# BCW-dot/PDE-based-Heston-Solver-GPU-accelerated

Hardware: AMD Instinct MI355X
Metric: grid-points x timesteps/sec (ADI sweep), 512x256 grid (higher is better)
Workload: dtype f64; 1 GPU; C2: European calls, Heston Douglas ADI, 512x256 grid, 1000 time steps, 256 strikes per GPU (85..115), HBM-resident inputs; m1=512, m2=256, instances_per_gpu=256, instances_total=256, parallelism=instances sharded over 1 GPU(s), no data-path collective

## Files before the change

pde_based_heston_solver_gpu_accelerated_amd/csrc/hadi_api.hip:

```cpp
#include "../../include/hadi.h"

#include <hip/hip_runtime.h>

#include <algorithm>
#include <climits>
#include <cmath>
#include <cstdarg>
#include <cstdio>
#include <cstdlib>
#include <cstring>
#include <string>
#include <vector>

#include "hadi_kernels.h"
#include "hadi_plan.h"

namespace {

struct DevBuf {
    void *p = nullptr;
    size_t cap = 0;
};

struct Ctx {
    int device = 0;
    hipStream_t stream = nullptr;
    hipEvent_t ev[4] = {nullptr, nullptr, nullptr, nullptr};
    std::vector<hipEvent_t> kev;
    int profiling = 0;
    int cu_count = 256;
    std::string name, arch;
    std::string err;
    hadi_timing timing{};
    DevBuf U, Y, LAM, U0, UT;
    DevBuf V, R1, C2;
    DevBuf rs_tab;
    DevBuf Uf, Yf;
    DevBuf scoef, b2row, rowc, a2i, pb, rinv, rwork, ipar, par8;
    DevBuf g_s, g_v, g_ds, g_dv;
    DevBuf src_v, src_dv, sel_a, sel_b, v0_i;
    DevBuf natU, natU0, natOut, prices, status;
    struct GraphEntry { std::string key; hipGraph_t graph; hipGraphExec_t exec; unsigned long long stamp; };
    std::vector<GraphEntry> graphs;
    unsigned long long graph_clock = 0;
    unsigned long long graph_captures = 0, graph_replays = 0, graph_drops = 0, graph_evictions = 0;
    int use_graph = 1;
    int graph_max_melems = 8;
    int use_small = 1;
    int small_seq = -1;
    int use_amp = 1;
    int device_vgrid = 1;
    int sub_batch = 1;
    int small_pairs = -1;
    int tile_il = 0;
    int col_prefetch = 0;
    int cs_strips = 1;
    int streams = 0;
    hipStream_t stream2 = nullptr;
    hipEvent_t fork_ev = nullptr, join_ev = nullptr;
    int last_nsub = 1;
    HadiTuning tune;
    hipEvent_t wait_ev = nullptr;
    DevBuf lm31;
    std::string last_path;
    DevBuf div_flag, div_amt, div_pct;
    DevBuf pay_mis;
    DevBuf order;
    int *err_host = nullptr, *err_dev = nullptr;
    char *pin = nullptr;
    size_t pin_cap = 0, pin_used = 0, pin_want = 0;
    int pin_dirty = 0;
    int debug_fault = 0;
    int team_launch = -1, team_failed = 0;
    DevBuf team;
};

struct DeviceGuard {
    int prev = -1;
    explicit DeviceGuard(int dev) {
        if (hipGetDevice(&prev) != hipSuccess) prev = -1;
        if (prev != dev) (void)hipSetDevice(dev);
        else prev = -1;
    }
    ~DeviceGuard() {
        if (prev >= 0) (void)hipSetDevice(prev);
    }
};

int fail(Ctx *c, int code, const char *fmt, ...) {
    char buf[512];
    va_list ap;
    va_start(ap, fmt);
    vsnprintf(buf, sizeof(buf), fmt, ap);
    va_end(ap);
    if (c) c->err = buf;
    return code;
}

#define HIP_TRY(c, call)                                                                          \
    do {                                                                                          \
        hipError_t e_ = (call);                                                                   \
        if (e_ != hipSuccess)                                                                     \
            return fail((c), HADI_ERR_HIP, "%s failed: %s (%s:%d)", #call, hipGetErrorString(e_), \
                        __FILE__, __LINE__);                                                      \
    } while (0)

void drop_graphs(Ctx *c) {
    for (auto &g : c->graphs) { (void)hipGraphExecDestroy(g.exec); (void)hipGraphDestroy(g.graph); }
    c->graph_drops += c->graphs.size();
    c->graphs.clear();
}

int ensure(Ctx *c, DevBuf &b, size_t bytes) {
    if (bytes <= b.cap) return HADI_OK;
    if (b.p) {
        HIP_TRY(c, hipStreamSynchronize(c->stream));
        drop_graphs(c);
        HIP_TRY(c, hipFree(b.p));
        b.p = nullptr;
        b.cap = 0;
    }
    const size_t want = bytes + bytes / 8 + 256;
    hipError_t e = hipMalloc(&b.p, want);
    if (e != hipSuccess) {
        b.p = nullptr;
        return fail(c, HADI_ERR_ALLOC, "hipMalloc(%zu bytes) failed: %s", want, hipGetErrorString(e));
    }
    b.cap = want;
    return HADI_OK;
}

template <class T>
T *ptr(DevBuf &b) {
    return static_cast<T *>(b.p);
}

void pin_rewind(Ctx *c) {
    if (c->pin_dirty && c->stream) (void)hipStreamSynchronize(c->stream);
    c->pin_dirty = 0;
    if (c->pin_want > c->pin_cap) {
        if (c->pin) (void)hipHostFree(c->pin);
        c->pin = nullptr; c->pin_cap = 0;
        const size_t want = c->pin_want + c->pin_want / 2 + 4096;
        void *q = nullptr;
        if (hipHostMalloc(&q, want, hipHostMallocDefault) == hipSuccess) { c->pin = static_cast<char *>(q); c->pin_cap = want; }
    }
    c->pin_used = 0;
    c->pin_want = 0;
}
void *pin_alloc(Ctx *c, size_t bytes) {
    const size_t need = (bytes + 63) & ~(size_t)63;
    c->pin_want += need;
    if (!c->pin || c->pin_used + need > c->pin_cap) return nullptr;
    void *q = c->pin + c->pin_used;
    c->pin_used += need;
    return q;
}
// ... 49 lines not shown
    int debug = 0, debug_step = 1;
};

template <int B, int G, int NG, int PD>
void launch_pass_a(const HadiPlan &pl, const HadiSweepArgs &a, int n, hipStream_t s, int mode = 0) {
    if (mode == 1)
        hipLaunchKernelGGL((hadi_pass_a<B, G, 4, NG, PD, false, 1>), dim3(pl.grid_a), dim3(64 * pl.W * G * NG), pl.smem_a, s, a, n);
    else if (mode == 2)
        hipLaunchKernelGGL((hadi_pass_a<B, G, 4, NG, PD, false, 2>), dim3(pl.grid_a), dim3(64 * pl.W * G * NG), pl.smem_a, s, a, n);
    else if (a.american)
        hipLaunchKernelGGL((hadi_pass_a<B, G, 4, NG, PD, true>), dim3(pl.grid_a), dim3(64 * pl.W * G * NG), pl.smem_a, s, a, n);
    else
        hipLaunchKernelGGL((hadi_pass_a<B, G, 4, NG, PD, false>), dim3(pl.grid_a), dim3(64 * pl.W * G * NG), pl.smem_a, s, a, n);
}

template <int B, int G, int NG, int PD>
void launch_pass_a_f32(const HadiPlan &pl, const HadiSweepArgs &a, int n, hipStream_t s) {
    const size_t ring_elems = (size_t)NG * ((PD + 1) * pl.W + 4) * pl.L.rowp;
    const size_t smem = pl.smem_a - ring_elems * (sizeof(double) - sizeof(float));
    hipLaunchKernelGGL((hadi_pass_a<B, G, 4, NG, PD, false, 0, float>), dim3(pl.grid_a), dim3(64 * pl.W * G * NG), smem, s, a, n);
}

template <int B, int G, int NG, int PD>
void launch_pass_a_amp(const HadiPlan &pl, const HadiSweepArgs &a, int n, hipStream_t s) {
    hipLaunchKernelGGL((hadi_pass_a<B, G, 4, NG, PD, 2>), dim3(pl.grid_a), dim3(64 * pl.W * G * NG),
                       pl.smem_a + (size_t)pl.L.rowp * sizeof(double), s, a, n);
}

template <class K>
hipError_t raise_lds_limit(K kernel) {
    return hipFuncSetAttribute(reinterpret_cast<const void *>(kernel), hipFuncAttributeMaxDynamicSharedMemorySize, 160 * 1024);
}
template <int B, int G, int NG, int PD>
hipError_t raise_pass_a() {
    hipError_t e = raise_lds_limit(hadi_pass_a<B, G, 4, NG, PD, false>);
    if (e == hipSuccess) e = raise_lds_limit(hadi_pass_a<B, G, 4, NG, PD, false, 1>);
    if (e == hipSuccess) e = raise_lds_limit(hadi_pass_a<B, G, 4, NG, PD, false, 2>);
    return e != hipSuccess ? e : raise_lds_limit(hadi_pass_a<B, G, 4, NG, PD, true>);
}
template <int B, int G, int NG, int PD, int SCH>
hipError_t raise_pass_a_sch() {
    hipError_t e = raise_lds_limit(hadi_pass_a_sch<B, G, 4, NG, PD, 1, SCH>);
    return e != hipSuccess ? e : raise_lds_limit(hadi_pass_a_sch<B, G, 4, NG, PD, 2, SCH>);
}
template <int SCH>
hipError_t raise_sch_lds_limits() {
    hipError_t e;
    if ((e = raise_pass_a_sch<1, 1, 1, 2, SCH>()) != hipSuccess) return e;
    if ((e = raise_pass_a_sch<2, 1, 1, 2, SCH>()) != hipSuccess) return e;
    if ((e = raise_pass_a_sch<4, 1, 1, 2, SCH>()) != hipSuccess) return e;
    if ((e = raise_pass_a_sch<8, 1, 1, 1, SCH>()) != hipSuccess) return e;
    if ((e = raise_pass_a_sch<8, 2, 1, 1, SCH>()) != hipSuccess) return e;
    if ((e = raise_lds_limit(hadi_pass_a_strip_sch<8, 1, 1, SCH>)) != hipSuccess) return e;
    if ((e = raise_lds_limit(hadi_pass_a_strip_sch<8, 1, 2, SCH>)) != hipSuccess) return e;
    if ((e = raise_lds_limit(hadi_pass_a_strip_sch<4, 1, 1, SCH>)) != hipSuccess) return e;
    if ((e = raise_lds_limit(hadi_pass_a_strip_sch<4, 1, 2, SCH>)) != hipSuccess) return e;
    if ((e = raise_lds_limit(hadi_pass_a_strip_sch<2, 1, 1, SCH>)) != hipSuccess) return e;
    if ((e = raise_lds_limit(hadi_pass_a_strip_sch<2, 1, 2, SCH>)) != hipSuccess) return e;
    return raise_lds_limit(hadi_pass_a_strip_sch<8, 2, 2, SCH>);
}
hipError_t raise_all_lds_limits() {
    hipError_t e;
    if ((e = raise_sch_lds_limits<HADI_SCH_MCS>()) != hipSuccess) return e;
    if ((e = raise_sch_lds_limits<HADI_SCH_HV>()) != hipSuccess) return e;
    if ((e = raise_pass_a<1, 1, 1, 2>()) != hipSuccess) return e;
    if ((e = raise_pass_a<2, 1, 1, 2>()) != hipSuccess) return e;
    if ((e = raise_pass_a<4, 1, 1, 2>()) != hipSuccess) return e;
    if ((e = raise_pass_a<8, 1, 1, 1>()) != hipSuccess) return e;
    if ((e = raise_pass_a<8, 2, 1, 1>()) != hipSuccess) return e;
    if ((e = raise_lds_limit(hadi_pass_a_strip<8, false>)) != hipSuccess) return e;
    if ((e = raise_lds_limit(hadi_pass_a_strip<8, true>)) != hipSuccess) return e;
    if ((e = raise_lds_limit(hadi_pass_a_strip<4, false>)) != hipSuccess) return e;
    if ((e = raise_lds_limit(hadi_pass_a_strip<4, true>)) != hipSuccess) return e;
    if ((e = raise_lds_limit(hadi_pass_a_strip<2, false>)) != hipSuccess) return e;
    if ((e = raise_lds_limit(hadi_pass_a_strip<2, true>)) != hipSuccess) return e;
    if ((e = raise_lds_limit(hadi_pass_a_strip<8, 2>)) != hipSuccess) return e;
    if ((e = raise_lds_limit(hadi_pass_a_strip<4, 2>)) != hipSuccess) return e;
    if ((e = raise_lds_limit(hadi_pass_a_strip<2, 2>)) != hipSuccess) return e;
    if ((e = raise_lds_limit(hadi_pass_a_pairs<0>)) != hipSuccess) return e;
    if ((e = raise_lds_limit(hadi_pass_a_pairs<1>)) != hipSuccess) return e;
    if ((e = raise_lds_limit(hadi_pass_a_pairs<2>)) != hipSuccess) return e;
    if ((e = raise_lds_limit(hadi_team_kernel<8>)) != hipSuccess) return e;
    if ((e = raise_lds_limit(hadi_team_kernel<4>)) != hipSuccess) return e;
    if ((e = raise_lds_limit(hadi_small_seq2_kernel<1>)) != hipSuccess) return e;
    if ((e = raise_lds_limit(hadi_small_seq2_kernel<2>)) != hipSuccess) return e;
    if ((e = raise_lds_limit(hadi_small_seq_kernel<1>)) != hipSuccess) return e;
    if ((e = raise_lds_limit(hadi_small_seq_kernel<2>)) != hipSuccess) return e;
    if ((e = raise_lds_limit(hadi_small_kernel<1, 4, false>)) != hipSuccess) return e;
    if ((e = raise_lds_limit(hadi_small_kernel<1, 4, true>)) != hipSuccess) return e;
    if ((e = raise_lds_limit(hadi_small_kernel<2, 4, false>)) != hipSuccess) return e;
    if ((e = raise_lds_limit(hadi_small_kernel<2, 4, true>)) != hipSuccess) return e;
    if ((e = raise_lds_limit(hadi_small_kernel<1, 8, false>)) != hipSuccess) return e;
    if ((e = raise_lds_limit(hadi_small_kernel<1, 8, true>)) != hipSuccess) return e;
    if ((e = raise_lds_limit(hadi_small_kernel<2, 8, false>)) != hipSuccess) return e;
    if ((e = raise_lds_limit(hadi_small_kernel<2, 8, true>)) != hipSuccess) return e;
    if ((e = raise_lds_limit(hadi_pass_b<8, false>)) != hipSuccess) return e;
    if ((e = raise_lds_limit(hadi_pass_b<8, true>)) != hipSuccess) return e;
    if ((e = raise_lds_limit(hadi_pass_b1<16, false>)) != hipSuccess) return e;
    if ((e = raise_lds_limit(hadi_pass_b2<16, double, HADI_B2_NPF(8)>)) != hipSuccess) return e;
    if ((e = raise_lds_limit(hadi_pass_b2<16, float, HADI_B2_NPF(4)>)) != hipSuccess) return e;
    if ((e = raise_lds_limit(hadi_pass_b<8, 2>)) != hipSuccess) return e;
    if ((e = raise_lds_limit(hadi_pass_b1<16, 2>)) != hipSuccess) return e;
    if ((e = raise_lds_limit(hadi_pass_a<1, 1, 4, 1, 2, 2>)) != hipSuccess) return e;
    if ((e = raise_lds_limit(hadi_pass_a<2, 1, 4, 1, 2, 2>)) != hipSuccess) return e;
    if ((e = raise_lds_limit(hadi_pass_a<4, 1, 4, 1, 2, 2>)) != hipSuccess) return e;
    if ((e = raise_lds_limit(hadi_pass_a<8, 1, 4, 1, 1, 2>)) != hipSuccess) return e;
    if ((e = raise_lds_limit(hadi_pass_a<8, 2, 4, 1, 1, 2>)) != hipSuccess) return e;
    if ((e = raise_lds_limit(hadi_pass_a_strip<8, false, float>)) != hipSuccess) return e;
    if ((e = raise_lds_limit(hadi_pass_a_strip<8, false, float, 2>)) != hipSuccess) return e;
    if ((e = raise_lds_limit(hadi_pass_a_strip<8, false, double, 2>)) != hipSuccess) return e;
    if ((e = raise_lds_limit(hadi_pass_a_strip<8, 1, double, 2>)) != hipSuccess) return e;
    if ((e = raise_lds_limit(hadi_pass_a_strip<8, 2, double, 2>)) != hipSuccess) return e;
    if ((e = raise_lds_limit(hadi_pass_b<8, false, float>)) != hipSuccess) return e;
    if ((e = raise_lds_limit(hadi_pass_b1<16, false, float>)) != hipSuccess) return e;
    if ((e = raise_lds_limit(hadi_pass_a<1, 1, 4, 1, 2, false, 0, float>)) != hipSuccess) return e;
    if ((e = raise_lds_limit(hadi_pass_a<2, 1, 4, 1, 2, false, 0, float>)) != hipSuccess) return e;
    if ((e = raise_lds_limit(hadi_pass_a<4, 1, 4, 1, 2, false, 0, float>)) != hipSuccess) return e;
    if ((e = raise_lds_limit(hadi_pass_a<8, 1, 4, 1, 1, false, 0, float>)) != hipSuccess) return e;
    if ((e = raise_lds_limit(hadi_pass_a<8, 2, 4, 1, 1, false, 0, float>)) != hipSuccess) return e;
    return raise_lds_limit(hadi_pass_b1<16, true>);
}

struct SubBatch { int off, cnt; HadiPlan pl; int lane; };
struct BatchPlan {
    std::vector<SubBatch> subs;
    bool two_streams = false;
    int fork_before = 0;
};
int plan_batches(Ctx *c, const SweepDesc &d, HadiPlan &pl, int state_bytes, bool seq_shape, BatchPlan &bp) {
    std::vector<SubBatch> &subs = bp.subs;
    bool &two_streams = bp.two_streams;
    int &fork_before = bp.fork_before;
    const bool no_strips = !(d.theta > 0.0) || d.r_d == d.r_f;
    auto plan_for = [&](int cnt, HadiPlan *q) {
        if (hadi_make_plan(d.m1, d.m2, cnt, 8 * c->cu_count, q, c->tune, state_bytes)) return 1;
        if (no_strips) q->use_strip = 0;
        return 0;
    };
    if (no_strips) pl.use_strip = 0;
    if (d.scheme == HADI_SCHEME_DOUGLAS && !d.debug && c->sub_batch && d.n > c->cu_count &&
        2ll * c->cu_count * pl.L.inst_stride * (long long)state_bytes >= (256ll << 20)) {
        const int cu = c->cu_count, full = d.n / cu, rem = d.n - full * cu;
        for (int k = 0; k < full; k++) subs.push_back(SubBatch{k * cu, cu, pl, 0});
        if (rem >= cu / 4) subs.push_back(SubBatch{full * cu, rem, pl, 0});
        else subs.back().cnt += rem;
        for (auto &sbt : subs)
            if (plan_for(sbt.cnt, &sbt.pl)) return fail(c, HADI_ERR_UNSUPPORTED, "plan failed");
        pl = subs[0].pl;
    } else {
        subs.push_back(SubBatch{0, d.n, pl, 0});
    }
    const bool streams_ok = d.scheme == HADI_SCHEME_DOUGLAS && !d.debug && !c->profiling && d.n >= 2 && !seq_shape;
    auto split_last = [&]() -> int {
        const SubBatch last = subs.back();
        const int h0 = (last.cnt + 1) / 2;
        subs.pop_back();
        subs.push_back(SubBatch{last.off, h0, last.pl, 0});
        subs.push_back(SubBatch{last.off + h0, last.cnt - h0, last.pl, 1});
        for (size_t k = subs.size() - 2; k < subs.size(); k++)
            if (plan_for(subs[k].cnt, &subs[k].pl)) return 1;
        return 0;
    };
    if (streams_ok && c->streams == 2) {
        if (subs.size() == 1) {
            if (split_last()) return fail(c, HADI_ERR_UNSUPPORTED, "plan failed");
        } else {
// ... 334 lines not shown
    sa.r_d = d.r_d; sa.r_f = d.r_f; sa.theta = d.theta;
    sa.scoef = ptr<double>(c->scoef); sa.b2row = ptr<double>(c->b2row); sa.rowc = ptr<double>(c->rowc);
    sa.a2i = ptr<double>(c->a2i); sa.pb = ptr<double>(c->pb); sa.rinv = ptr<double>(c->rinv);
    sa.rwork = ptr<double>(c->rwork); sa.ipar = ptr<HadiInstPar>(c->ipar);
    hipLaunchKernelGGL(hadi_setup_kernel, dim3(d.n), dim3(256), 0, s, sa);

    const size_t tot = (size_t)L.inst_stride * d.n;
    hipLaunchKernelGGL(hadi_pack_kernel, dim3(grid1d(tot)), dim3(256), 0, s, L, d.n, d.n_src, d.d_natU, ptr<double>(c->U));
    if (american) {
        hipLaunchKernelGGL(hadi_pack_kernel, dim3(grid1d(tot)), dim3(256), 0, s, L, d.n, d.n_src,
                           d.d_natU0 ? d.d_natU0 : d.d_natU, ptr<double>(c->U0));
        HIP_TRY(c, hipMemsetAsync(c->LAM.p, 0, st, s));
        if ((rc = ensure(c, c->pay_mis, sizeof(int) * n))) return rc;
        HIP_TRY(c, hipMemsetAsync(c->pay_mis.p, 0, sizeof(int) * n, s));
        hipLaunchKernelGGL(hadi_payoff_shape_kernel, dim3(grid1d(tot)), dim3(256), 0, s, L, d.n, ptr<double>(c->U0), ptr<int>(c->pay_mis));
    }
    bool amp = false;
    const bool takes_small_path = c->use_small && !c->profiling && !cs && !f32 && !d.debug && (american ? pl.smem_small_am : pl.smem_small_eu) > 0;
    if (american && c->use_amp && !cs && !takes_small_path && !d.debug && !seq_shape) {
        std::vector<int> mis(d.n);
        HIP_TRY(c, hipMemcpyAsync(mis.data(), c->pay_mis.p, sizeof(int) * n, hipMemcpyDeviceToHost, s));
        HIP_TRY(c, hipStreamSynchronize(s));
        amp = true;
        for (int k = 0; k < d.n; k++) amp = amp && mis[k] == 0;
    }
    HIP_TRY(c, hipGetLastError());

    if (f32) {
        hipLaunchKernelGGL(hadi_narrow_kernel, dim3(grid1d(tot)), dim3(256), 0, s, L, ptr<double>(c->U), ptr<float>(c->Uf), tot);
        HIP_TRY(c, hipMemsetAsync(c->Yf.p, 0, st / 2, s));
    }
    HadiSweepArgs a;
    a.U = ptr<double>(c->U); a.Y = ptr<double>(c->Y);
    if (f32) {
        a.U = reinterpret_cast<double *>(c->Uf.p);
        a.Y = reinterpret_cast<double *>(c->Yf.p);
    }
    a.LAM = american ? ptr<double>(c->LAM) : nullptr;
    a.U0 = american ? ptr<double>(c->U0) : nullptr;
    a.pay_mis = american ? ptr<int>(c->pay_mis) : nullptr;
    a.scoef = ptr<double>(c->scoef); a.b2row = ptr<double>(c->b2row); a.rowc = ptr<double>(c->rowc);
    a.pb = ptr<double>(c->pb); a.rinv = ptr<double>(c->rinv); a.ipar = ptr<HadiInstPar>(c->ipar);
    a.L = L; a.n_inst = d.n; a.R = pl.R; a.ntiles = pl.ntiles; a.ctiles = pl.ctiles; a.btpw = pl.btpw; a.bgroups = pl.bgroups;
    a.american = american ? 1 : 0; a.pos_m1 = pl.pos_m1;
    a.tile_il = c->tile_il;
    a.RS = pl.RS; a.sblocks = pl.sblocks;
    a.err = c->err_dev; a.debug = c->debug_fault;
    a.R1 = (cs || pl.row_seq) ? ptr<double>(c->R1) : nullptr;
    a.C2 = cs ? ptr<double>(c->C2) : nullptr;
    a.rs_tab = pair_tab ? ptr<double>(c->rs_tab) : nullptr;
    HadiSweepArgs av = a;
    if (cs) av.U = ptr<double>(c->V);

    const bool prof = c->profiling != 0 && !d.debug;
    if (prof) {
        const size_t need = (size_t)4 * d.Nmax * nsub;
        while (c->kev.size() < need) {
            hipEvent_t e;
            HIP_TRY(c, hipEventCreate(&e));
            c->kev.push_back(e);
        }
    }
    auto shift = [&](HadiSweepArgs x, int o, int cnt, const HadiPlan &sp) {
        x.n_inst = cnt; x.R = sp.R; x.ntiles = sp.ntiles; x.ctiles = sp.ctiles; x.btpw = sp.btpw; x.bgroups = sp.bgroups;
        x.RS = sp.RS; x.sblocks = sp.sblocks;
        const size_t so = (size_t)o * L.inst_stride;
        if (f32) {
            x.U = reinterpret_cast<double *>(reinterpret_cast<float *>(x.U) + so);
            x.Y = reinterpret_cast<double *>(reinterpret_cast<float *>(x.Y) + so);
        } else {
            x.U += so;
            x.Y += so;
        }
        if (x.LAM) x.LAM += so;
        if (x.U0) x.U0 += so;
        if (x.pay_mis) x.pay_mis += o;
        if (x.R1) x.R1 += so;
        if (x.C2) x.C2 += so;
        if (x.rs_tab) x.rs_tab += (size_t)o * L.nrows * 128;
        x.scoef += (size_t)o * pl.n_scoef; x.b2row += (size_t)o * pl.n_b2row; x.rowc += (size_t)o * pl.n_rowc;
        x.pb += (size_t)o * pl.n_pb; x.rinv += (size_t)o * pl.n_rinv; x.ipar += o;
        return x;
    };
    const HadiSweepArgs a_all = a, av_all = av;
    bool forked = false;
    auto enqueue_body = [&](hipStream_t q0) -> int {
      const int n_first = d.debug ? d.debug_step : 1, n_last = d.debug ? d.debug_step : d.Nmax;
      for (int sb = 0; sb < nsub; sb++) {
        if (two_streams && sb == fork_before) {
            HIP_TRY(c, hipEventRecord(c->fork_ev, q0));
            HIP_TRY(c, hipStreamWaitEvent(c->stream2, c->fork_ev, 0));
            forked = true;
        }
        hipStream_t q = (two_streams && subs[sb].lane) ? c->stream2 : q0;
        const int o = subs[sb].off, nsb = subs[sb].cnt;
        const HadiPlan &pl = subs[sb].pl;
        const size_t so = (size_t)o * L.inst_stride;
        const HadiSweepArgs a = shift(a_all, o, nsb, pl), av = shift(av_all, o, nsb, pl);
        const size_t tot = (size_t)L.inst_stride * nsb, st = tot * sizeof(double);
        double *const Ub = ptr<double>(c->U) + so, *const LAMb = american ? ptr<double>(c->LAM) + so : nullptr;
        double *const U0b = american ? ptr<double>(c->U0) + so : nullptr, *const UTb = dividend ? ptr<double>(c->UT) + so : nullptr;
        const int ev0 = 4 * sb * d.Nmax;
        if (pair_tab && pl.use_strip) {
            HadiSweepArgs at = a;
            at.U = Ub;
            const size_t sm = (size_t)4 * HADI_STRIP_NS(8, 2, 8) * L.rowp * sizeof(double) + ((size_t)4 * 64 * 8 * 2 + (size_t)4 * 16) * sizeof(double);
            hipLaunchKernelGGL((hadi_pass_a_strip<8, 0, double, 2, 3>), dim3(pl.grid_as), dim3(512), sm, q, at, 1);
        }
        for (int nstep = n_first; nstep <= n_last; nstep++) {
            const bool xstep = amp && (nstep == 1 || (have_div && div_step[nstep]));
            if (xstep && nstep > 1)
                hipLaunchKernelGGL(hadi_am_materialise_kernel, dim3(grid1d(tot)), dim3(256), 0, q, L, nsb, a.ipar, U0b, Ub, LAMb, pl.pos_m1);
            if (have_div && div_step[nstep]) {
                if (f32)
                    hipLaunchKernelGGL(hadi_widen_kernel, dim3(grid1d(tot)), dim3(256), 0, q, L, reinterpret_cast<const float *>(a.U), Ub, tot);
                HIP_TRY(c, hipMemcpyAsync(UTb, Ub, st, hipMemcpyDeviceToDevice, q));
                const size_t npts = (size_t)nsb * L.nrows * (L.m1 + 1);
                hipLaunchKernelGGL(hadi_dividend_kernel, dim3(grid1d(npts)), dim3(256), 0, q, L, nsb, a.ipar,
                                   d.d_vec_s + (size_t)o * (L.m1 + 1), UTb, Ub, ptr<int>(c->div_flag) + (size_t)o * flag_stride,
                                   flag_stride, nstep, ptr<double>(c->div_amt), ptr<double>(c->div_pct));
                if (f32)
                    hipLaunchKernelGGL(hadi_narrow_kernel, dim3(grid1d(tot)), dim3(256), 0, q, L, Ub, reinterpret_cast<float *>(a.U), tot);
            }
            if (prof) HIP_TRY(c, hipEventRecord(c->kev[ev0 + 4 * (nstep - 1) + 0], q));
            const PassEnv env{pl, L, nsb, q, nstep, american, amp, xstep, f32, c->col_prefetch, c->cs_strips, d.scheme};
            auto row_pass = [&](const HadiSweepArgs &ar, int mode) { launch_row_pass(env, ar, mode); };
            auto col_pass = [&](const HadiSweepArgs &ar) { launch_col_pass(env, ar); };
            if (d.debug == 2) {
                HIP_TRY(c, hipMemcpyAsync(a.Y, a.U, f32 ? st / 2 : st, hipMemcpyDeviceToDevice, q));
                col_pass(a);
                break;
            }
            row_pass(a, cs ? 1 : 0);
            if (d.debug == 1) break;
            if (prof) {
                HIP_TRY(c, hipEventRecord(c->kev[ev0 + 4 * (nstep - 1) + 1], q));
                HIP_TRY(c, hipEventRecord(c->kev[ev0 + 4 * (nstep - 1) + 2], q));
            }
            col_pass(cs ? av : a);
            if (prof) HIP_TRY(c, hipEventRecord(c->kev[ev0 + 4 * (nstep - 1) + 3], q));
            if (cs) {
                row_pass(av, 2);
                col_pass(a);
            }
            if (xstep)
                hipLaunchKernelGGL(hadi_am_dematerialise_kernel, dim3(grid1d(tot)), dim3(256), 0, q, L, nsb, a.ipar, U0b, Ub, LAMb);
        }
        if (amp)
            hipLaunchKernelGGL(hadi_am_materialise_kernel, dim3(grid1d(tot)), dim3(256), 0, q, L, nsb, a.ipar, U0b, Ub, LAMb, pl.pos_m1);
      }
      return HADI_OK;
    };
    auto enqueue_loop = [&](hipStream_t q0) -> int {
      forked = false;
      const int rcb = enqueue_body(q0);
      if (forked) {
          const hipError_t e1 = hipEventRecord(c->join_ev, c->stream2);
          const hipError_t e2 = e1 == hipSuccess ? hipStreamWaitEvent(q0, c->join_ev, 0) : e1;
          if (!rcb && e2 != hipSuccess) return fail(c, HADI_ERR_HIP, "joining the second stream failed: %s", hipGetErrorString(e2));
      }
      return rcb;
    };

    const size_t smem_small = american ? pl.smem_small_am : pl.smem_small_eu;
    const bool seq = takes_small_path && !american && (c->small_seq > 0 || (c->small_seq < 0 && d.n > c->cu_count));
    const size_t smem_seq = (size_t)hadi_small_seq_layout(L.m1, L.nrows).total * sizeof(double);
    const bool seq2 = seq && L.nrows <= 32 && 2 * smem_seq <= (size_t)160 * 1024 &&
                      (c->small_pairs > 0 || (c->small_pairs < 0 && d.n > 2 * c->cu_count && 2 * d.n <= 9 * c->cu_count));
    if (takes_small_path) {
        {
            char buf[192];
            if (seq2)
                std::snprintf(buf, sizeof buf, "hadi_small_seq2_kernel<%d>: whole time loop in one launch, two instances per wavefront, lines solved sequentially in LDS (2 x %zu B)", L.B, smem_seq);
            else if (seq)
                std::snprintf(buf, sizeof buf, "hadi_small_seq_kernel<%d>: whole time loop in one launch, one wavefront per instance, lines solved sequentially in LDS (%zu B)", L.B, smem_seq);
            else
                std::snprintf(buf, sizeof buf, "hadi_small_kernel<%d,%d,%s>: whole time loop in one launch, instance resident in LDS (%zu B)", L.B,
                              (c->tune.small_waves ? c->tune.small_waves : (d.n <= 2 * c->cu_count ? 8 : 4)) == 8 ? 8 : 4, american ? "AM" : "EU", smem_small);
            c->last_path = buf;
        }
        HadiSmallArgs sm;
        sm.div_flag = nullptr; sm.div_amounts = nullptr; sm.div_pcts = nullptr; sm.vec_s = d.d_vec_s; sm.Nmax = d.Nmax;
        sm.order = nullptr;
        if (!d.uniform_steps) {
            std::vector<int> order(d.n);
            for (int k = 0; k < d.n; k++) order[k] = k;
            std::stable_sort(order.begin(), order.end(), [&](int x, int y) {
                return d.par8[(size_t)x * 8 + 5] > d.par8[(size_t)y * 8 + 5];
            });
            if ((rc = ensure(c, c->order, sizeof(int) * n))) return rc;
            if ((rc = stage_to_device(c, c->order.p, order.data(), sizeof(int) * n))) return rc;
            sm.order = ptr<int>(c->order);
        }
        sm.flag_stride = flag_stride;
        if (have_div) {
            sm.div_flag = ptr<int>(c->div_flag); sm.div_amounts = ptr<double>(c->div_amt); sm.div_pcts = ptr<double>(c->div_pct);
        }
        HIP_TRY(c, hipEventRecord(c->ev[1], s));
        const int sw = c->tune.small_waves ? c->tune.small_waves : (d.n <= 2 * c->cu_count ? 8 : 4);
        if (seq2) {
            if (L.B == 1) hipLaunchKernelGGL((hadi_small_seq2_kernel<1>), dim3((d.n + 1) / 2), dim3(64), 2 * smem_seq, s, a, sm);
            else hipLaunchKernelGGL((hadi_small_seq2_kernel<2>), dim3((d.n + 1) / 2), dim3(64), 2 * smem_seq, s, a, sm);
        } else if (seq) {
            if (L.B == 1) hipLaunchKernelGGL((hadi_small_seq_kernel<1>), dim3(d.n), dim3(64), smem_seq, s, a, sm);
            else hipLaunchKernelGGL((hadi_small_seq_kernel<2>), dim3(d.n), dim3(64), smem_seq, s, a, sm);
        } else if (sw == 8) {
            if (L.B == 1) {
                if (american) hipLaunchKernelGGL((hadi_small_kernel<1, 8, true>), dim3(d.n), dim3(512), smem_small, s, a, sm);
                else hipLaunchKernelGGL((hadi_small_kernel<1, 8, false>), dim3(d.n), dim3(512), smem_small, s, a, sm);
            } else {
                if (american) hipLaunchKernelGGL((hadi_small_kernel<2, 8, true>), dim3(d.n), dim3(512), smem_small, s, a, sm);
                else hipLaunchKernelGGL((hadi_small_kernel<2, 8, false>), dim3(d.n), dim3(512), smem_small, s, a, sm);
            }
        } else if (L.B == 1) {
            if (american) hipLaunchKernelGGL((hadi_small_kernel<1, 4, true>), dim3(d.n), dim3(256), smem_small, s, a, sm);
            else hipLaunchKernelGGL((hadi_small_kernel<1, 4, false>), dim3(d.n), dim3(256), smem_small, s, a, sm);
        } else {
            if (american) hipLaunchKernelGGL((hadi_small_kernel<2, 4, true>), dim3(d.n), dim3(256), smem_small, s, a, sm);
            else hipLaunchKernelGGL((hadi_small_kernel<2, 4, false>), dim3(d.n), dim3(256), smem_small, s, a, sm);
        }
        HIP_TRY(c, hipGetLastError());
        HIP_TRY(c, hipEventRecord(c->ev[2], s));
        return HADI_OK;
    }

    c->last_path = describe_streaming_path(c, pl, bp, american, amp, d.scheme, f32);
    c->last_nsub = nsub;
    HIP_TRY(c, hipEventRecord(c->ev[1], s));
    const bool team_shape = d.n <= 8 && L.G == 1 && (L.B == 8 || L.B == 4) && L.P <= 8 && !seq_shape && (d.variant == HADI_EU || d.variant == HADI_DIV) && !cs && !f32 &&
                            !d.debug && !prof && d.theta > 0.0 && d.r_d != d.r_f && c->cu_count == 256;
    const bool pinned = c->tune.strip >= 0 || c->tune.row_tile > 0 || c->tune.col_groups > 0 || c->tune.strip_blocks > 0;
    if (team_shape && (c->team_launch > 0 || (c->team_launch < 0 && !c->team_failed && !pinned))) {
        if ((rc = ensure(c, c->team, 512 * sizeof(int)))) return rc;
        HIP_TRY(c, hipMemsetAsync(c->team.p, 0, 512 * sizeof(int), s));
        HadiTeamArgs ta;
        ta.form = ptr<int>(c->team); ta.bar = ptr<int>(c->team) + 64; ta.nb = c->cu_count / 8; ta.N = d.Nmax;
        ta.div_flag = have_div ? ptr<int>(c->div_flag) : nullptr; ta.flag_stride = flag_stride;
        ta.div_amounts = have_div ? ptr<double>(c->div_amt) : nullptr; ta.div_pcts = have_div ? ptr<double>(c->div_pct) : nullptr;
        ta.vec_s = d.d_vec_s;
        ta.stamps = reinterpret_cast<unsigned long long *>(ptr<int>(c->team) + 384);
        const size_t smem = ((size_t)4 * 64 * L.B + hadi_pb_mf_doubles(L.P) + (size_t)L.P * HADI_LC * HADI_PBW +
                             (have_div ? (size_t)(L.m1 + 2) + (size_t)8 * L.rowp : 0)) * sizeof(double) + 64;
        if (L.B == 8) hipLaunchKernelGGL((hadi_team_kernel<8>), dim3(c->cu_count), dim3(512), smem, s, a, ta);
        else hipLaunchKernelGGL((hadi_team_kernel<4>), dim3(c->cu_count), dim3(512), smem, s, a, ta);
        HIP_TRY(c, hipGetLastError());
        HIP_TRY(c, hipStreamSynchronize(s));
        const int deverr = __atomic_exchange_n(c->err_host, 0, __ATOMIC_ACQ_REL);
        if (!deverr) {
            char buf[200];
            std::snprintf(buf, sizeof buf, "hadi_team_kernel<%d>: whole time loop in one launch, every instance resident in one XCD's L2 (teams of %d blocks)",
                          L.B, ta.nb);
            c->last_path = buf;
            HIP_TRY(c, hipEventRecord(c->ev[2], s));
            return HADI_OK;
        }
        if (deverr & ~HADI_DEVERR_TEAM) __atomic_fetch_or(c->err_host, deverr & ~HADI_DEVERR_TEAM, __ATOMIC_RELAXED);
        c->team_failed = 1;
        hipLaunchKernelGGL(hadi_pack_kernel, dim3(grid1d(tot)), dim3(256), 0, s, L, d.n, d.n_src, d.d_natU, ptr<double>(c->U));
        HIP_TRY(c, hipMemsetAsync(c->Y.p, 0, st, s));
        c->last_path += " (after a failed instance-resident launch)";
    }
    const bool graphable = c->use_graph && !prof && !d.debug && (long long)d.n * L.inst_stride <= ((long long)c->graph_max_melems << 20);
    if (graphable) {
        std::string key;
        auto put = [&](const void *p_, size_t nbytes) { key.append(static_cast<const char *>(p_), nbytes); };
        {
            const void *pa[HADI_SWEEP_ARGS_NPTRS], *pv[HADI_SWEEP_ARGS_NPTRS];
            hadi_sweep_args_ptrs(a, pa);
            hadi_sweep_args_ptrs(av, pv);
            const void *own[] = {c->U.p, c->LAM.p, c->U0.p, c->UT.p, c->div_flag.p, c->div_amt.p, c->div_pct.p, d.d_vec_s};
            const int ints[] = {a.debug, a.L.m1, a.L.m2, a.L.B, a.L.G, a.L.P, a.n_inst, a.R, a.ntiles, a.ctiles, a.btpw, a.bgroups,
                                a.american, a.pos_m1, d.scheme, d.prec, (int)amp, (int)two_streams, nsub, pl.row_seq, pl.col_seq, pl.use_pairs, pl.use_strip, pl.RS, pl.sblocks, pl.grid_as, pl.grid_a, pl.grid_b, pl.block_b, pl.W, (int)pl.smem_a, (int)pl.smem_b};
            put(pa, sizeof(pa));
            put(pv, sizeof(pv));
            put(own, sizeof(own));
            put(ints, sizeof(ints));
        }
        for (const auto &sbt : subs) {
            const HadiPlan &q = sbt.pl;
            const int geo[] = {c->col_prefetch, c->cs_strips, c->tile_il, sbt.lane, fork_before, sbt.off, sbt.cnt, q.R, q.ntiles, q.grid_a, (int)q.smem_a, q.use_strip, q.use_pairs, q.RS, q.sblocks, q.grid_as,
                               (int)q.smem_as, q.ctiles, q.btpw, q.bgroups, q.grid_b, q.block_b, (int)q.smem_b, q.row_seq, q.col_seq, q.W, q.NG, q.PD};
            put(geo, sizeof(geo));
        }
        put(&d.Nmax, sizeof(int)); put(&d.dt0, sizeof(double));
        put(&d.variant, sizeof(int));
        if (have_div) {
            put(&flag_stride, sizeof(int));
            put(div_step.data(), div_step.size());
        }
        Ctx::GraphEntry *hit = nullptr;
        for (auto &g : c->graphs)
            if (g.key == key) { hit = &g; break; }
        if (!hit) {
            if (c->graphs.size() >= 8) {
                size_t lru = 0;
                for (size_t k = 1; k < c->graphs.size(); k++)
                    if (c->graphs[k].stamp < c->graphs[lru].stamp) lru = k;
                (void)hipGraphExecDestroy(c->graphs[lru].exec);
                (void)hipGraphDestroy(c->graphs[lru].graph);
                c->graphs.erase(c->graphs.begin() + lru);
                c->graph_evictions++;
            }
            hipGraph_t graph = nullptr;
            hipGraphExec_t exec = nullptr;
            HIP_TRY(c, hipStreamBeginCapture(s, hipStreamCaptureModeThreadLocal));
            const int rcl = enqueue_loop(s);
            hipError_t ec = hipStreamEndCapture(s, &graph);
            if (rcl || ec != hipSuccess) {
                if (graph) (void)hipGraphDestroy(graph);
                if (rcl) return rcl;
            }
            HIP_TRY(c, ec);
            HIP_TRY(c, hipGraphInstantiate(&exec, graph, nullptr, nullptr, 0));
            c->graphs.push_back(Ctx::GraphEntry{key, graph, exec, 0});
            hit = &c->graphs.back();
            c->graph_captures++;
        } else {
            c->graph_replays++;
        }
        hit->stamp = ++c->graph_clock;
        HIP_TRY(c, hipGraphLaunch(hit->exec, s));
    } else {
        const int rcl = enqueue_loop(s);
        if (rcl) return rcl;
    }
    HIP_TRY(c, hipGetLastError());
    HIP_TRY(c, hipEventRecord(c->ev[2], s));
    if (f32)
        hipLaunchKernelGGL(hadi_widen_kernel, dim3(grid1d(tot)), dim3(256), 0, s, L, ptr<float>(c->Uf), ptr<double>(c->U), tot);
    return HADI_OK;
}

int finish_timing(Ctx *c, const SweepDesc &d, const HadiPlan &pl) {
    hipStream_t s = c->stream;
    HIP_TRY(c, hipEventRecord(c->ev[3], s));
    HIP_TRY(c, hipStreamSynchronize(s));
    c->pin_dirty = 0;
    const int deverr = __atomic_exchange_n(c->err_host, 0, __ATOMIC_ACQ_REL);
    float ms = 0;
    hadi_timing &t = c->timing;
    t = hadi_timing{};
    HIP_TRY(c, hipEventElapsedTime(&ms, c->ev[0], c->ev[1])); t.setup_ms = ms;
    HIP_TRY(c, hipEventElapsedTime(&ms, c->ev[1], c->ev[2])); t.sweep_ms = ms;
    HIP_TRY(c, hipEventElapsedTime(&ms, c->ev[2], c->ev[3])); t.finish_ms = ms;
    long long ps = 0;
    const long long m = (long long)(d.m1 + 1) * (d.m2 + 1);
    for (int k = 0; k < d.n; k++) ps += m * (long long)d.par8[(size_t)k * 8 + 5];
    t.point_steps = ps;
    if (c->profiling && !d.debug && (int)c->kev.size() >= 4 * d.Nmax * c->last_nsub) {
        for (int k = 0; k < d.Nmax * c->last_nsub; k++) {
            HIP_TRY(c, hipEventElapsedTime(&ms, c->kev[4 * k], c->kev[4 * k + 1])); t.pass_a_ms += ms;
            HIP_TRY(c, hipEventElapsedTime(&ms, c->kev[4 * k + 2], c->kev[4 * k + 3])); t.pass_b_ms += ms;
        }
        t.pass_a_launches = (long long)d.Nmax * c->last_nsub;
        t.pass_b_launches = (long long)d.Nmax * c->last_nsub;
    }
    (void)pl;
    if (deverr)
        return fail(c, HADI_ERR_INTERNAL, "device-side failure 0x%x during the sweep%s: the results of this call are invalid", deverr,
                    (deverr & HADI_DEVERR_RENDEZVOUS) ? " (a pair rendezvous of a two-wavefront row ran out of polls)" : "");
    return HADI_OK;
}

int to_device(Ctx *c, int memspace, const double *src, size_t count, DevBuf &buf, const double **out) {
// ... 351 lines not shown
        case HADI_ERR_NOT_ON_GRID: return "S_0 is not a grid node";
        case HADI_ERR_NO_DEVICE: return "no usable gfx950 GPU (libhadi has no CPU path)";
        case HADI_ERR_ALLOC: return "device allocation failed";
        case HADI_ERR_INTERNAL: return "device-side failure reported by a kernel (results invalid)";
        default: return "unknown";
    }
}

int hadi_create(hadi_ctx **out, int device_id) {
    if (!out) return HADI_ERR_INVALID;
    *out = nullptr;
    int count = 0;
    if (hipGetDeviceCount(&count) != hipSuccess || count < 1) return HADI_ERR_NO_DEVICE;
    if (device_id < 0 || device_id >= count) return HADI_ERR_INVALID;
    DeviceGuard guard(device_id);
    hipDeviceProp_t prop;
    if (hipGetDeviceProperties(&prop, device_id) != hipSuccess) return HADI_ERR_HIP;
    if (std::strncmp(prop.gcnArchName, "gfx950", 6) != 0) return HADI_ERR_NO_DEVICE;
    Ctx *c = new Ctx;
    c->device = device_id;
    c->cu_count = prop.multiProcessorCount > 0 ? prop.multiProcessorCount : 256;
    c->name = prop.name;
    c->arch = prop.gcnArchName;
    bool ok = hipStreamCreateWithFlags(&c->stream, hipStreamNonBlocking) == hipSuccess;
    ok = ok && hipStreamCreateWithFlags(&c->stream2, hipStreamNonBlocking) == hipSuccess;
    ok = ok && hipEventCreateWithFlags(&c->fork_ev, hipEventDisableTiming) == hipSuccess;
    ok = ok && hipEventCreateWithFlags(&c->join_ev, hipEventDisableTiming) == hipSuccess;
    ok = ok && raise_all_lds_limits() == hipSuccess;
    for (auto &e : c->ev) ok = ok && hipEventCreate(&e) == hipSuccess;
    ok = ok && hipEventCreateWithFlags(&c->wait_ev, hipEventDisableTiming) == hipSuccess;
    ok = ok && hipHostMalloc(reinterpret_cast<void **>(&c->err_host), 64, hipHostMallocMapped | hipHostMallocCoherent) == hipSuccess;
    if (ok) {
        c->pin_want = (size_t)1 << 20;
        pin_rewind(c);
        *c->err_host = 0;
        ok = hipHostGetDevicePointer(reinterpret_cast<void **>(&c->err_dev), c->err_host, 0) == hipSuccess;
    }
    if (!ok) {
        release_handle(c);
        return HADI_ERR_HIP;
    }
    *out = reinterpret_cast<hadi_ctx *>(c);
    return HADI_OK;
}

int hadi_destroy(hadi_ctx *ctx) {
    Ctx *c = reinterpret_cast<Ctx *>(ctx);
    if (!c) return HADI_OK;
    DeviceGuard guard(c->device);
    release_handle(c);
    return HADI_OK;
}

const char *hadi_last_error(const hadi_ctx *ctx) {
    const Ctx *c = reinterpret_cast<const Ctx *>(ctx);
    return c ? c->err.c_str() : "null handle";
}

int hadi_set_profiling(hadi_ctx *ctx, int enabled) {
    Ctx *c = reinterpret_cast<Ctx *>(ctx);
    if (!c) return HADI_ERR_INVALID;
    c->profiling = enabled ? 1 : 0;
    return HADI_OK;
}

int hadi_set_tuning(hadi_ctx *ctx, const char *key, int value) {
    Ctx *c = reinterpret_cast<Ctx *>(ctx);
    if (!c || !key) return HADI_ERR_INVALID;
    if (!std::strcmp(key, "graph")) c->use_graph = value ? 1 : 0;
    else if (!std::strcmp(key, "small_grid")) c->use_small = value ? 1 : 0;
    else if (!std::strcmp(key, "small_seq")) c->small_seq = value < 0 ? -1 : (value ? 1 : 0);
    else if (!std::strcmp(key, "american_p")) c->use_amp = value ? 1 : 0;
    else if (!std::strcmp(key, "device_vgrid")) c->device_vgrid = value ? 1 : 0;
    else if (!std::strcmp(key, "sub_batch")) c->sub_batch = value ? 1 : 0;
    else if (!std::strcmp(key, "small_pairs")) c->small_pairs = value < 0 ? -1 : (value ? 1 : 0);
    else if (!std::strcmp(key, "streams")) c->streams = value == 2 ? 2 : (value == 1 ? 1 : 0);
    else if (!std::strcmp(key, "col_prefetch")) c->col_prefetch = value ? 1 : 0;
    else if (!std::strcmp(key, "cs_strips")) c->cs_strips = (value >= 0 && value <= 3) ? value : 1;
    else if (!std::strcmp(key, "graph_max_melems")) c->graph_max_melems = value > 0 ? value : 0;
    else if (!std::strcmp(key, "tile_interleave")) c->tile_il = value ? 1 : 0;
    else if (!std::strcmp(key, "strip")) c->tune.strip = value < 0 ? -1 : (value ? 1 : 0);
    else if (!std::strcmp(key, "debug_fault")) c->debug_fault = value;
    else if (!std::strcmp(key, "team_launch")) { c->team_launch = value < 0 ? -1 : (value ? 1 : 0); c->team_failed = 0; }
    else if (!std::strcmp(key, "row_tile")) c->tune.row_tile = value > 0 ? value : 0;
    else if (!std::strcmp(key, "strip_blocks")) c->tune.strip_blocks = value > 0 ? value : 0;
    else if (!std::strcmp(key, "pair_strips")) c->tune.pair_strips = value < 0 ? -1 : (value ? 1 : 0);
    else if (!std::strcmp(key, "col_groups")) c->tune.col_groups = value > 0 ? value : 0;
    else if (!std::strncmp(key, "model_", 6)) {
        struct { const char *k; int HadiTuning::*f; } const tab[] = {
            {"model_strip_row_ns", &HadiTuning::strip_row_ns}, {"model_ring_row_ps", &HadiTuning::ring_row_ps}, {"model_ring_fixed_ns", &HadiTuning::ring_fixed_ns},
            {"model_pstrip_row_ns", &HadiTuning::pstrip_row_ns}, {"model_pring_row_ps", &HadiTuning::pring_row_ps}, {"model_pring_fixed_ns", &HadiTuning::pring_fixed_ns}};
        bool hit = false;
        for (auto &e : tab)
            if (!std::strcmp(key, e.k)) { if (value < 1) return fail(c, HADI_ERR_INVALID, "%s must be positive", key); c->tune.*(e.f) = value; hit = true; }
        if (!hit) return fail(c, HADI_ERR_INVALID, "unknown tuning key '%s'", key);
    }
    else if (!std::strcmp(key, "small_waves")) {
        if (value != 0 && value != 4 && value != 8) return fail(c, HADI_ERR_INVALID, "small_waves must be 0, 4 or 8");
        c->tune.small_waves = value;
    } else if (!std::strcmp(key, "graph_captures") || !std::strcmp(key, "graph_replays") || !std::strcmp(key, "graph_drops") ||
               !std::strcmp(key, "graph_evictions")) {
        return fail(c, HADI_ERR_INVALID, "'%s' is a read-only counter", key);
    } else return fail(c, HADI_ERR_INVALID, "unknown tuning key '%s'", key);
    return HADI_OK;
}

int hadi_get_tuning(const hadi_ctx *ctx, const char *key, int *value) {
    const Ctx *c = reinterpret_cast<const Ctx *>(ctx);
    if (!c || !key || !value) return HADI_ERR_INVALID;
    if (!std::strcmp(key, "graph")) *value = c->use_graph;
    else if (!std::strcmp(key, "small_grid")) *value = c->use_small;
    else if (!std::strcmp(key, "small_seq")) *value = c->small_seq;
    else if (!std::strcmp(key, "american_p")) *value = c->use_amp;
    else if (!std::strcmp(key, "device_vgrid")) *value = c->device_vgrid;
    else if (!std::strcmp(key, "sub_batch")) *value = c->sub_batch;
    else if (!std::strcmp(key, "small_pairs")) *value = c->small_pairs;
    else if (!std::strcmp(key, "streams")) *value = c->streams;
    else if (!std::strcmp(key, "col_prefetch")) *value = c->col_prefetch;
    else if (!std::strcmp(key, "cs_strips")) *value = c->cs_strips;
    else if (!std::strcmp(key, "graph_max_melems")) *value = c->graph_max_melems;
    else if (!std::strcmp(key, "tile_interleave")) *value = c->tile_il;
    else if (!std::strcmp(key, "strip")) *value = c->tune.strip;
    else if (!std::strcmp(key, "debug_fault")) *value = c->debug_fault;
    else if (!std::strcmp(key, "team_launch")) *value = c->team_failed ? -2 : c->team_launch;
    else if (!std::strcmp(key, "row_tile")) *value = c->tune.row_tile;
    else if (!std::strcmp(key, "strip_blocks")) *value = c->tune.strip_blocks;
    else if (!std::strcmp(key, "pair_strips")) *value = c->tune.pair_strips;
    else if (!std::strcmp(key, "col_groups")) *value = c->tune.col_groups;
    else if (!std::strcmp(key, "model_strip_row_ns")) *value = c->tune.strip_row_ns;
    else if (!std::strcmp(key, "model_ring_row_ps")) *value = c->tune.ring_row_ps;
    else if (!std::strcmp(key, "model_ring_fixed_ns")) *value = c->tune.ring_fixed_ns;
    else if (!std::strcmp(key, "model_pstrip_row_ns")) *value = c->tune.pstrip_row_ns;
    else if (!std::strcmp(key, "model_pring_row_ps")) *value = c->tune.pring_row_ps;
    else if (!std::strcmp(key, "model_pring_fixed_ns")) *value = c->tune.pring_fixed_ns;
    else if (!std::strcmp(key, "small_waves")) *value = c->tune.small_waves;
    else if (!std::strcmp(key, "graph_captures")) *value = (int)std::min<unsigned long long>(c->graph_captures, INT_MAX);
    else if (!std::strcmp(key, "graph_replays")) *value = (int)std::min<unsigned long long>(c->graph_replays, INT_MAX);
    else if (!std::strcmp(key, "graph_drops")) *value = (int)std::min<unsigned long long>(c->graph_drops, INT_MAX);
    else if (!std::strcmp(key, "graph_evictions")) *value = (int)std::min<unsigned long long>(c->graph_evictions, INT_MAX);
    else return HADI_ERR_INVALID;
    return HADI_OK;
}

int hadi_wait_stream(hadi_ctx *ctx, void *producer_stream) {
    Ctx *c = reinterpret_cast<Ctx *>(ctx);
    if (!c) return HADI_ERR_INVALID;
    DeviceGuard guard(c->device);
    HIP_TRY(c, hipEventRecord(c->wait_ev, static_cast<hipStream_t>(producer_stream)));
    HIP_TRY(c, hipStreamWaitEvent(c->stream, c->wait_ev, 0));
    return HADI_OK;
}

int hadi_get_timing(const hadi_ctx *ctx, hadi_timing *out) {
    const Ctx *c = reinterpret_cast<const Ctx *>(ctx);
    if (!c || !out) return HADI_ERR_INVALID;
    *out = c->timing;
    return HADI_OK;
}

int hadi_device_info(const hadi_ctx *ctx, char *name, int name_len, int *compute_units, char *arch, int arch_len) {
    const Ctx *c = reinterpret_cast<const Ctx *>(ctx);
    if (!c) return HADI_ERR_INVALID;
    if (name && name_len > 0) std::snprintf(name, name_len, "%s", c->name.c_str());
    if (arch && arch_len > 0) std::snprintf(arch, arch_len, "%s", c->arch.c_str());
    if (compute_units) *compute_units = c->cu_count;
    return HADI_OK;
}

int hadi_describe_last_sweep(const hadi_ctx *ctx, char *buf, int len) {
    const Ctx *c = reinterpret_cast<const Ctx *>(ctx);
    if (!c || !buf || len <= 0) return HADI_ERR_INVALID;
    std::snprintf(buf, len, "%s", c->last_path.c_str());
    return HADI_OK;
}

void *hadi_stream(hadi_ctx *ctx) {
    Ctx *c = reinterpret_cast<Ctx *>(ctx);
    return c ? (void *)c->stream : nullptr;
}

int hadi_make_grid(int m1, double S, double S_0, double K, double cc, int m2, double V, double V_0, double d,
                   double *vec_s, double *vec_v, double *delta_s, double *delta_v) {
    if (m1 < 1 || m2 < 1 || !vec_s || !vec_v || !delta_s || !delta_v) return HADI_ERR_INVALID;
    const double lo = std::asinh(-K / cc);
    const double Delta_xi = (1.0 / m1) * (std::asinh((S - K) / cc) - lo);
    for (int i = 0; i <= m1; i++) vec_s[i] = K + cc * std::sinh(lo + i * Delta_xi);
    sorted_insert_drop_largest(vec_s, m1 + 1, S_0);
    for (int i = 0; i < m1; i++) delta_s[i] = vec_s[i + 1] - vec_s[i];
    build_v(m2, V_0, V, d, vec_v, delta_v);
    return HADI_OK;
}

int hadi_rebuild_variance(int m2, double V_0_new, double V, double d, double *vec_v, double *delta_v) {
    if (m2 < 1 || !vec_v || !delta_v) return HADI_ERR_INVALID;
    build_v(m2, V_0_new, V, d, vec_v, delta_v);
    return HADI_OK;
}

int hadi_find_s_index(int m1, const double *vec_s, double S_0) {
    for (int i = 0; i <= m1; i++)
        if (std::fabs(vec_s[i] - S_0) < 1e-10) return i;
    return -1;
}

int hadi_find_v_index(int m2, const double *vec_v, double V_0) {
    for (int i = 0; i <= m2; i++)
        if (std::fabs(vec_v[i] - V_0) < 1e-10) return i;
// ... 148 lines not shown
```

pde_based_heston_solver_gpu_accelerated_amd/csrc/hadi_kernels.h:

```cpp
#pragma once
#include "hadi_core.h"

#include "hadi_k_common.h"
#include "hadi_k_row_ring.h"
#include "hadi_k_row_strip.h"
#include "hadi_k_col.h"
#include "hadi_k_team.h"
#include "hadi_k_small.h"
#include "hadi_k_seq.h"
#include "hadi_k_aux.h"
```

Before: 160.3 billion point-steps/s.

## Fuse all ADI time steps into one persistent per-instance resident kernel

Adds a persistent kernel, hadi_sweep_resident<8>, that runs every time step for one instance inside a single block. It alternates the row (pass A) and column (pass B) phases, separated by block-level barriers and a memory drain. The kernel is used by default for Douglas European f64 shapes when the instance count fits in the CU count and no geometry tuning is pinned. This removes thousands of per-step kernel launches and the grid-level dependencies between them. In exchange it limits parallelism to one block per instance and relies on intra-block syncs to make global memory writes visible between phases.

```diff
diff --git a/pde_based_heston_solver_gpu_accelerated_amd/csrc/hadi_api.hip b/pde_based_heston_solver_gpu_accelerated_amd/csrc/hadi_api.hip
--- a/pde_based_heston_solver_gpu_accelerated_amd/csrc/hadi_api.hip
+++ b/pde_based_heston_solver_gpu_accelerated_amd/csrc/hadi_api.hip
@@ -73,6 +73,7 @@
     int debug_fault = 0;
     int team_launch = -1, team_failed = 0;
     DevBuf team;
+    int resident_sweep = -1;
 };
 
 struct DeviceGuard {
@@ -288,6 +289,7 @@
     if ((e = raise_lds_limit(hadi_pass_a_pairs<2>)) != hipSuccess) return e;
     if ((e = raise_lds_limit(hadi_team_kernel<8>)) != hipSuccess) return e;
     if ((e = raise_lds_limit(hadi_team_kernel<4>)) != hipSuccess) return e;
+    if ((e = raise_lds_limit(hadi_sweep_resident<8>)) != hipSuccess) return e;
     if ((e = raise_lds_limit(hadi_small_seq2_kernel<1>)) != hipSuccess) return e;
     if ((e = raise_lds_limit(hadi_small_seq2_kernel<2>)) != hipSuccess) return e;
     if ((e = raise_lds_limit(hadi_small_seq_kernel<1>)) != hipSuccess) return e;
@@ -788,6 +790,14 @@
         x.pb += (size_t)o * pl.n_pb; x.rinv += (size_t)o * pl.n_rinv; x.ipar += o;
         return x;
     };
+    const bool geo_pinned = c->tune.strip >= 0 || c->tune.row_tile > 0 || c->tune.col_groups > 0 || c->tune.strip_blocks > 0;
+    const bool resident_shape = (c->resident_sweep > 0 || (c->resident_sweep < 0 && !geo_pinned)) && d.scheme == HADI_SCHEME_DOUGLAS &&
+                                d.variant == HADI_EU && !f32 && L.B == 8 && L.G == 1 && L.P <= 8 && !seq_shape && d.theta > 0.0 &&
+                                d.r_d != d.r_f && !d.debug && !c->debug_fault && !prof;
+    auto resident = [&](const SubBatch &sbt) {
+        return resident_shape && sbt.pl.use_strip && !sbt.pl.use_pairs && sbt.pl.sblocks == 1 && sbt.cnt <= c->cu_count &&
+               hadi_plan_row_idle(sbt.pl, sbt.cnt, c->cu_count) < HADI_TWO_STREAM_IDLE;
+    };
     const HadiSweepArgs a_all = a, av_all = av;
     bool forked = false;
     auto enqueue_body = [&](hipStream_t q0) -> int {
@@ -812,6 +822,10 @@
             at.U = Ub;
             const size_t sm = (size_t)4 * HADI_STRIP_NS(8, 2, 8) * L.rowp * sizeof(double) + ((size_t)4 * 64 * 8 * 2 + (size_t)4 * 16) * sizeof(double);
             hipLaunchKernelGGL((hadi_pass_a_strip<8, 0, double, 2, 3>), dim3(pl.grid_as), dim3(512), sm, q, at, 1);
+        }
+        if (resident(subs[sb])) {
+            hipLaunchKernelGGL((hadi_sweep_resident<8>), dim3(pl.grid_as), dim3(64 * HADI_STRIP_WAVES(8)), std::max(pl.smem_as, pl.smem_b), q, a, n_last);
+            continue;
         }
         for (int nstep = n_first; nstep <= n_last; nstep++) {
             const bool xstep = amp && (nstep == 1 || (have_div && div_step[nstep]));
@@ -931,6 +945,15 @@
     }
 
     c->last_path = describe_streaming_path(c, pl, bp, american, amp, d.scheme, f32);
+    {
+        int nres = 0;
+        for (const auto &sbt : subs) nres += resident(sbt) ? 1 : 0;
+        if (nres == nsub)
+            c->last_path += "; both passes of every step in one launch: hadi_sweep_resident<8> (one block per instance, all column tiles)";
+        else if (nres)
+            c->last_path += "; both passes of every step in one launch for " + std::to_string(nres) +
+                            " sub-batches of one round: hadi_sweep_resident<8> (one block per instance, all column tiles), the others streaming";
+    }
     c->last_nsub = nsub;
     HIP_TRY(c, hipEventRecord(c->ev[1], s));
     const bool team_shape = d.n <= 8 && L.G == 1 && (L.B == 8 || L.B == 4) && L.P <= 8 && !seq_shape && (d.variant == HADI_EU || d.variant == HADI_DIV) && !cs && !f32 &&
@@ -985,7 +1008,8 @@
         for (const auto &sbt : subs) {
             const HadiPlan &q = sbt.pl;
             const int geo[] = {c->col_prefetch, c->cs_strips, c->tile_il, sbt.lane, fork_before, sbt.off, sbt.cnt, q.R, q.ntiles, q.grid_a, (int)q.smem_a, q.use_strip, q.use_pairs, q.RS, q.sblocks, q.grid_as,
-                               (int)q.smem_as, q.ctiles, q.btpw, q.bgroups, q.grid_b, q.block_b, (int)q.smem_b, q.row_seq, q.col_seq, q.W, q.NG, q.PD};
+                               (int)q.smem_as, q.ctiles, q.btpw, q.bgroups, q.grid_b, q.block_b, (int)q.smem_b, q.row_seq, q.col_seq, q.W, q.NG, q.PD,
+                               resident(sbt) ? 1 : 0};
             put(geo, sizeof(geo));
         }
         put(&d.Nmax, sizeof(int)); put(&d.dt0, sizeof(double));
@@ -1503,6 +1527,7 @@
     else if (!std::strcmp(key, "strip")) c->tune.strip = value < 0 ? -1 : (value ? 1 : 0);
     else if (!std::strcmp(key, "debug_fault")) c->debug_fault = value;
     else if (!std::strcmp(key, "team_launch")) { c->team_launch = value < 0 ? -1 : (value ? 1 : 0); c->team_failed = 0; }
+    else if (!std::strcmp(key, "resident_sweep")) c->resident_sweep = value < 0 ? -1 : (value ? 1 : 0);
     else if (!std::strcmp(key, "row_tile")) c->tune.row_tile = value > 0 ? value : 0;
     else if (!std::strcmp(key, "strip_blocks")) c->tune.strip_blocks = value > 0 ? value : 0;
     else if (!std::strcmp(key, "pair_strips")) c->tune.pair_strips = value < 0 ? -1 : (value ? 1 : 0);
@@ -1544,6 +1569,7 @@
     else if (!std::strcmp(key, "strip")) *value = c->tune.strip;
     else if (!std::strcmp(key, "debug_fault")) *value = c->debug_fault;
     else if (!std::strcmp(key, "team_launch")) *value = c->team_failed ? -2 : c->team_launch;
+    else if (!std::strcmp(key, "resident_sweep")) *value = c->resident_sweep;
     else if (!std::strcmp(key, "row_tile")) *value = c->tune.row_tile;
     else if (!std::strcmp(key, "strip_blocks")) *value = c->tune.strip_blocks;
     else if (!std::strcmp(key, "pair_strips")) *value = c->tune.pair_strips;
diff --git a/pde_based_heston_solver_gpu_accelerated_amd/csrc/hadi_k_resident.h b/pde_based_heston_solver_gpu_accelerated_amd/csrc/hadi_k_resident.h
--- /dev/null
+++ b/pde_based_heston_solver_gpu_accelerated_amd/csrc/hadi_k_resident.h
@@ -0,0 +1,117 @@
+#pragma once
+
+
+HADI_DEV HADI_FORCEINLINE unsigned hadi_resident_tid() {
+#if defined(HADI_EMU)
+    return threadIdx.x;
+#else
+    unsigned t = threadIdx.x;
+    asm volatile("" : "+v"(t));
+    return t;
+#endif
+}
+#if defined(HADI_EMU)
+#define HADI_RESIDENT_TID
+#else
+#define HADI_RESIDENT_TID const struct { unsigned x; } threadIdx = {hadi_resident_tid()};
+#endif
+
+template <int B>
+HADI_DEV HADI_FORCEINLINE void hadi_resident_row_phase(const HadiSweepArgs &a, int n) {
+    HADI_RESIDENT_TID
+    constexpr int AMER = 0, G = 1, MODE = 0, SCH = HADI_SCH_CS;
+    typedef double T;
+#include "hadi_k_row_strip_body.h"
+}
+
+HADI_DEV HADI_FORCEINLINE void hadi_resident_col_phase(const HadiSweepArgs &a, int inst) {
+    HADI_DYN_SMEM(double, smem);
+    HADI_RESIDENT_TID
+    HadiPassBCtx c;
+    c.lane = threadIdx.x & 63;
+    c.wave = HADI_UNIFORM((int)(threadIdx.x >> 6));
+    c.P = a.L.P;
+    const int P = c.P, cnt = a.ctiles;
+    if (c.wave >= P) {
+        __syncthreads();
+        if (P > 1) {
+            for (int t = 0; t < cnt; t++) {
+                __syncthreads();
+                if (HADI_PB_MF) __syncthreads();
+            }
+        }
+        return;
+    }
+    const HadiInstPar ip = a.ipar[inst];
+    c.nrows = a.L.nrows;
+    c.rowp = a.L.rowp;
+    c.ja = c.wave * HADI_LC;
+    c.Yi = a.Y + (size_t)inst * a.L.inst_stride;
+    c.Ui = a.U + (size_t)inst * a.L.inst_stride;
+    c.Yb = hadi_make_buf(c.Yi, (size_t)a.L.inst_stride * sizeof(double));
+    c.Ub = hadi_make_buf(c.Ui, (size_t)a.L.inst_stride * sizeof(double));
+    c.Li = nullptr; c.Lb = hadi_make_buf(nullptr, 0); c.P0i = nullptr; c.pay1d = 0;
+    c.american = 0; c.debug = a.debug;
+    c.pos_m1 = a.pos_m1;
+    c.tabl = nullptr;
+    HadiTileSet ts;
+    ts.first = 0; ts.stride = 1; ts.nfull_mine = a.L.rowp >> 6; ts.short_tile = ts.nfull_mine; ts.cnt = cnt;
+    auto tile = [&](int i) { return hadi_pb_tile(ts, i); };
+#if defined(HADI_STAMPS) && !defined(HADI_EMU)
+    unsigned long long stamp_store_[32] = {0};
+    c.stamp_acc_ = stamp_store_;
+#endif
+    double ya[HADI_LC], yb[HADI_LC], yc[HADI_LC];
+    hadi_pb_load<double>(c, tile(0), ya);
+    hadi_pb_load_table(c, a.pb + ((size_t)inst * a.L.nrows_pad + c.ja) * HADI_PBW);
+    hadi_pb_setup_lds<HADI_PB_MF != 0>(c, smem, a.rinv + (size_t)inst * 16 * P * P, 2);
+    c.inv_dt = 1.0 / ip.dt;
+    c.dt = ip.dt;
+    __syncthreads();
+    if (1 < cnt) hadi_pb_load<double>(c, tile(1), yb);
+    for (int i = 0; i < cnt; i += 3) {
+        if (i + 2 < cnt) hadi_pb_load<double>(c, tile(i + 2), yc);
+        hadi_pb_solve_store<0, double>(c, tile(i), i & 1, ya, 0);
+        if (i + 1 < cnt) {
+            if (i + 3 < cnt) hadi_pb_load<double>(c, tile(i + 3), ya);
+            hadi_pb_solve_store<0, double>(c, tile(i + 1), (i + 1) & 1, yb, 0);
+        }
+        if (i + 2 < cnt) {
+            if (i + 4 < cnt) hadi_pb_load<double>(c, tile(i + 4), yb);
+            hadi_pb_solve_store<0, double>(c, tile(i + 2), (i + 2) & 1, yc, 0);
+        }
+    }
+}
+
+HADI_DEV HADI_FORCEINLINE void hadi_resident_drain() {
+#if !defined(HADI_EMU)
+    asm volatile("s_waitcnt vmcnt(0)" ::: "memory");
+#endif
+    __syncthreads();
+}
+
+HADI_DEV HADI_FORCEINLINE HadiSweepArgs hadi_resident_args(const HadiSweepArgs &a) {
+#if defined(__HIP_DEVICE_COMPILE__)
+    (void)a;
+    typedef const __attribute__((address_space(4))) HadiSweepArgs *HadiKargPtr;
+    HadiKargPtr p = (HadiKargPtr)__builtin_amdgcn_kernarg_segment_ptr();
+    asm volatile("" : "+s"(p));
+    return *p;
+#else
+    return a;
+#endif
+}
+
+template <int B>
+__global__ void __launch_bounds__(64 * HADI_STRIP_WAVES(B), 2) hadi_sweep_resident(HadiSweepArgs a, int N) {
+    static_assert(B == 8, "one wavefront per v-row of 8 nodes per lane");
+    const int inst = hadi_xcd_remap(blockIdx.x, gridDim.x);
+    if (inst >= a.n_inst) return;
+    const int Ni = a.ipar[inst].N < N ? a.ipar[inst].N : N;
+    for (int n = 1; n <= Ni; n++) {
+        hadi_resident_row_phase<B>(hadi_resident_args(a), n);
+        hadi_resident_drain();
+        hadi_resident_col_phase(hadi_resident_args(a), inst);
+        hadi_resident_drain();
+    }
+}
diff --git a/pde_based_heston_solver_gpu_accelerated_amd/csrc/hadi_kernels.h b/pde_based_heston_solver_gpu_accelerated_amd/csrc/hadi_kernels.h
--- a/pde_based_heston_solver_gpu_accelerated_amd/csrc/hadi_kernels.h
+++ b/pde_based_heston_solver_gpu_accelerated_amd/csrc/hadi_kernels.h
@@ -6,6 +6,7 @@
 #include "hadi_k_row_strip.h"
 #include "hadi_k_col.h"
 #include "hadi_k_team.h"
+#include "hadi_k_resident.h"
 #include "hadi_k_small.h"
 #include "hadi_k_seq.h"
 #include "hadi_k_aux.h"
```

Result: faster. 177.7 billion point-steps/s (median of 6 runs) (+10.9%).
